# kianoosh-j/CL_MultiView_Stereo

Hardware: AMD Instinct MI355X
Metric: Mpix/s depth (1080p, 128 depth hyp, 5 views) + depth L1 vs ref (higher is better)
Workload: dtype i8 (NCC: 8-bit intensities as int8 v_dot4 operands, i32 window sums, f32 costs; SLIC / superpixel SAD / refinement in f32 with the reference's f64 promotions)

## Files before the change

cl_multiview_stereo_amd/csrc/ncc_mfma.hip:

```cpp
#include <type_traits>

#include "ncc_common.h"

#ifndef MVS_MFMA_SPLIT
#define MVS_MFMA_SPLIT 1
#endif

namespace mvs {
namespace ncc {
namespace {

struct alignas(128) NccMRec {
  int txmax, tymax;
  int bhp, shp;
  int colo[16];
  int pad0[2];
  unsigned off_lo, off_hi;
  int pad[8];
};
static_assert(sizeof(NccMRec) == 4 * kRecWords, "one 128-B record per (chunk, neighbour)");

template <int K, int BW, bool TAIL, bool VERT, int NDB, int NB, int DBG = 0>
__global__ __launch_bounds__(512) __attribute__((amdgpu_waves_per_eu(4))) void k_ncc_mfma(
    const uint2* __restrict__ stats, const uint2* __restrict__ pk, const NccMRec* __restrict__ plan, NccArgs a,
    WtaOut wo) {
  static_assert(NDB == 1 || NDB == 2, "one or two 16-level blocks per chunk");
  static_assert(K == 5 || K == 7, "5 x 5 or 7 x 7 windows");
  static_assert(K == 5 || !VERT, "K = 7: horizontal lists only");
  static_assert(VERT || NB == 2 || NB == 3, "the horizontal form is double- or triple-buffered");
  static_assert(VERT || NDB == (K == 5 ? 2 : 1), "horizontal chunks: 32 levels (K = 5), 16 (K = 7: A takes 32 VGPRs)");
  constexpr int R = K / 2, NW = 8, TH = 8, DC = 16 * NDB, NK = K * K;
  constexpr int XB = K == 5 ? 2 : 4, NYB = K == 5 ? TH / 4 : 1, NBL = XB * NYB, MF = K == 5 ? 1 : 2;
  constexpr int BXW = 8 / XB;
  constexpr int BWP = BW + 1;
  constexpr bool SPLIT = MVS_MFMA_SPLIT;
  extern __shared__ __align__(16) uint8_t smem[];
  const int nbuf = (a.pk_pairs + a.st_pairs) * BWP;
  u32x4* nbase = (u32x4*)smem;
  const int band_bytes = max(NB * nbuf * 16, 3 * 16 * kMfMergeStride * 4);
  float* rsn_l = (float*)(smem + band_bytes);
  float* srl = rsn_l + 64 * TH;
  short* colo_l = (short*)(srl + 64 * TH);

  const int tid = threadIdx.x, lane = tid & 63, wave = __builtin_amdgcn_readfirstlane(tid >> 6);
  const int W = a.W, H = a.H;
  const int Hp2 = (H + 1) >> 1;
  const long Pv = (long)W * Hp2 * 2;
  const long P = (long)W * H;
  const int bid = blockIdx.x, grp = bid & 7;
  const int tg = grp * a.tiles_per_xcd + (bid >> 3);
  if (tg >= a.ntiles * a.nref) return;
  const int ref = tg / a.ntiles, tile = tg - ref * a.ntiles;
  const int x0 = (tile % a.tiles_x) * 64;
  const int y0 = (tile / a.tiles_x) * TH;
  const int nn = a.nn[ref], T = a.nch * nn;
  const NccMRec* rec = plan + a.plan[ref];

  const int bhp = K == 5 ? (TH + 4) / 2 : (TH + 8) / 2, shp = TH / 2;
  const long pk_row = 2L * W * min(max((y0 >> 1) - (K == 5 ? 1 : 2) + wave, 0), Hp2 - 1);
  const long st_row = 2L * W * min(max(y0 / 2 + wave, 0), Hp2 - 1);
  struct StepInfo {
    int tx, shp;
    unsigned lo, hi;
  };
  auto load_info = [&](int t, int n) -> StepInfo {
    const NccMRec& e = rec[t];
    return StepInfo{e.txmax, e.shp, e.off_lo, e.off_hi};
  };
  const int lane_x = x0 + lane;
  auto stage_h = [&](const StepInfo& e, int b) {
    if (DBG == 2) return;
    const int span = (e.shp >> 16) & 0xff, nblk = (span + 127) >> 6;
    const unsigned long long vo = (unsigned long long)e.hi << 32 | e.lo;
    u32x4* npk = nbase + b * nbuf + ((wave & 1) ? (e.shp >> 24) : 0);
    u32x4* nst = nbase + b * nbuf + a.pk_pairs * BWP + ((K == 7 && wave >= 2) ? ((e.shp << 16) >> 24) : 0);
    if (wave < shp) {
      const __amdgpu_buffer_rsrc_t rp = buf_rsrc((const char*)pk + vo + 8 * pk_row, 16 * W);
      const __amdgpu_buffer_rsrc_t rs = buf_rsrc((const char*)stats + vo + 8 * st_row, 16 * W);
      for (int cb = 0; cb < nblk; cb++) {
        const int c0 = min(cb * 64, span);
        const int voff = 16 * min(max(lane_x - e.tx + c0, 0), W - 1);
        __builtin_amdgcn_raw_ptr_buffer_load_lds(rp, (lds_ptr_t)(npk + wave * BWP + c0), 16, voff, 0, 0, 0);
        __builtin_amdgcn_raw_ptr_buffer_load_lds(rs, (lds_ptr_t)(nst + wave * BWP + c0), 16, voff, 0, 0, 0);
      }
    } else if (wave < bhp) {
      const __amdgpu_buffer_rsrc_t rp = buf_rsrc((const char*)pk + vo + 8 * pk_row, 16 * W);
      for (int cb = 0; cb < nblk; cb++) {
        const int c0 = min(cb * 64, span);
        const int voff = 16 * min(max(lane_x - e.tx + c0, 0), W - 1);
        __builtin_amdgcn_raw_ptr_buffer_load_lds(rp, (lds_ptr_t)(npk + wave * BWP + c0), 16, voff, 0, 0, 0);
      }
    }
  };
  auto stage = [&](int t, int n, int b) {
    if (DBG == 2) return;
    const NccMRec& e = rec[t];
    const int span = (e.shp >> 16) & 0xff, nblk = (span + 127) >> 6;
    const long vo = (long)a.view[ref][n] * Pv;
    u32x4* npk = nbase + b * nbuf;
    u32x4* nst = npk + a.pk_pairs * BWP;
    const int xb0 = x0 - e.txmax + lane;
    if constexpr (!VERT) {
      for (int cb = 0; cb < nblk; cb++) {
        const int c0 = min(cb * 64, span);
        const int xx = min(max(xb0 + c0, 0), W - 1);
        if (wave < bhp) glds_b128(pk + vo + pk_row + 2 * xx, npk + wave * BWP + c0);
        if (wave < shp) glds_b128(stats + vo + st_row + 2 * xx, nst + wave * BWP + c0);
      }
    } else {
      const int ebh = e.bhp, esh = e.shp & 0xff;
      const int pm0 = (y0 - R - e.tymax) >> 1, sm0 = (y0 - e.tymax) >> 1;
      for (int cb = 0; cb < nblk; cb++) {
        const int c0 = min(cb * 64, span);
        const int xx = min(max(xb0 + c0, 0), W - 1);
        const uint2* gpk = pk + vo + 2 * xx;
        const uint2* gst = stats + vo + 2 * xx;
        for (int i = wave; i < ebh; i += NW) glds_b128(gpk + 2L * W * min(max(pm0 + i, 0), Hp2 - 1), npk + i * BWP + c0);
        for (int i = wave; i < esh; i += NW) glds_b128(gst + 2L * W * min(max(sm0 + i, 0), Hp2 - 1), nst + i * BWP + c0);
      }
    }
  };

  for (int i = tid; i < T * DC / 2; i += NW * 64) ((int*)colo_l)[i] = rec[i / (DC / 2)].colo[i % (DC / 2)];
  auto nmod = [&](int v) { return v >= nn ? v - nn : v; };
  StepInfo cur{}, nxt{}, nx2{};
  if constexpr (!VERT) {
    cur = load_info(0, 0);
    if (T > 1) nxt = load_info(1, nmod(1 % nn));
    if (NB == 3 && T > 2) nx2 = load_info(2, nmod(2 % nn));
    stage_h(cur, 0);
    if (NB == 3 && T > 1) stage_h(nxt, 1);
  } else {
    stage(0, 0, 0);
  }
  const long zo = (long)a.z[ref] * Pv;
  const int zp0 = min(max((y0 >> 1) - (K == 5 ? 1 : 2), 0), Hp2 - 1);
  const __amdgpu_buffer_rsrc_t rz = buf_rsrc((const char*)pk + 8 * (zo + 2L * W * zp0), 16 * W * min(Hp2 - zp0, 8));
  for (int o = wave; o < TH; o += NW) {
    const int x = x0 + lane, y = y0 + o;
    const int xoff = 16 * min(x, W - 1);
    int s1 = 0, s2 = 0;
#pragma unroll
    for (int k = 0; k < 2 * R + 1; k++) {
      const int yc = min(max(y - R + k, 0), H - 1);
      const u32x2 v = __builtin_amdgcn_raw_buffer_load_b64(rz, xoff, 16 * W * ((yc >> 1) - zp0) + 8 * (yc & 1), 0);
      const unsigned lo = v.x, hi = v.y & (K == 5 ? 0xffu : 0xffffffu);
      s1 = dot4(lo, 0x01010101u, dot4(hi, 0x01010101u, s1));
      s2 = dot4(lo, lo, dot4(hi, hi, s2));
    }
    const bool valid = x - R >= 0 && x + R < W && y - R >= 0 && y + R < H;
    const int var = NK * s2 - s1 * s1;
    srl[lane * TH + o] = !valid ? __int_as_float(0x7fc00000) : (var != 0 ? 1.0f / sqrtf((float)var) : 0.0f);
    rsn_l[lane * TH + o] = -(float)s1;
  }
  i32x4 A[NBL][MF];
  {
    const int mA = lane & 15, g = lane >> 4;
    const int xxA = K == 5 ? mA >> 2 : mA >> 3, yyA = K == 5 ? mA & 3 : mA & 7;
    const unsigned long long cm = (K == 5 ? 0xFFFFFFFFFFull : 0xFFFFFFFFFFFFFFull) << (8 * xxA);
    const unsigned cm_lo = (unsigned)cm, cm_hi = (unsigned)(cm >> 32);
    unsigned msk[MF][4];
#pragma unroll
    for (int mf = 0; mf < MF; mf++)
#pragma unroll
      for (int h = 0; h < 2; h++) {
        const int rr = 2 * (g + 4 * mf) + h;
        const bool in = (unsigned)(rr - yyA - (K == 5 ? 0 : 1)) <= (unsigned)(K - 1);
        msk[mf][2 * h] = in ? cm_lo : 0u;
        msk[mf][2 * h + 1] = in ? cm_hi : 0u;
      }
    constexpr int NPR = K == 5 ? NYB : MF;
    int roff[NPR];
#pragma unroll
    for (int i = 0; i < NPR; i++) {
      const int pr = min(max((K == 5 ? (y0 >> 1) - 1 + 2 * i : (y0 >> 1) - 2 + 4 * i) + g, 0), Hp2 - 1);
      roff[i] = 16 * W * (pr - zp0);
    }
#pragma unroll
    for (int xb = 0; xb < XB; xb++) {
      const int xcol = min(x0 + 8 * wave + BXW * xb, W - 1);
#pragma unroll
      for (int yb = 0; yb < NYB; yb++)
#pragma unroll
        for (int mf = 0; mf < MF; mf++) {
          const u32x4 v = __builtin_amdgcn_raw_buffer_load_b128(rz, roff[K == 5 ? yb : mf], 16 * xcol, 0);
          A[xb * NYB + yb][mf] = i32x4{(int)(v.x & msk[mf][0]), (int)(v.y & msk[mf][1]), (int)(v.z & msk[mf][2]),
                                       (int)(v.w & msk[mf][3])};
        }
    }
  }
  auto pcol = [&](int xb, int g) { return BXW * xb + (K == 5 ? g : g >> 1); };
  auto prow = [&](int yb, int g) { return K == 5 ? 4 * yb : 4 * (g & 1); };
  __syncthreads();

  float E[NBL][NDB][4];
  float wv0[NBL][4], wv1[NBL][4];
  unsigned wi0p[NBL][2];
#pragma unroll
  for (int k = 0; k < NBL; k++) {
#pragma unroll
    for (int r = 0; r < 4; r++) {
      wv0[k][r] = kWtaInit;
      wv1[k][r] = kWtaInit;
    }
    wi0p[k][0] = wi0p[k][1] = 0xffffffffu;
  }
  const i32x4 bias = i32x4{kMagicI, kMagicI, kMagicI, kMagicI};

  auto fold = [&](int c) {
    const int ln = lane_now();
    float kill[NDB];
#pragma unroll
    for (int db = 0; db < NDB; db++) kill[db] = 0.0f;
    if (TAIL && c == a.nch - 1)
#pragma unroll
      for (int db = 0; db < NDB; db++) kill[db] = c * DC + 16 * db + (ln & 15) >= a.D ? INFINITY : 0.0f;
#pragma unroll
    for (int xb = 0; xb < XB; xb++)
#pragma unroll
      for (int yb = 0; yb < NYB; yb++) {
        const int kb = xb * NYB + yb;
        const f32x4 sq = *(const f32x4*)(srl + (8 * wave + pcol(xb, ln >> 4)) * TH + prow(yb, ln >> 4));
        const int dl0 = c * DC + (ln & 15);
        const unsigned d0 = (unsigned)dl0 * 0x10001u, d1 = (unsigned)(dl0 + 16) * 0x10001u;
#pragma unroll
        for (int r = 0; r < 4; r += 2) {
          f32x2 cst[NDB];
#pragma unroll
          for (int db = 0; db < NDB; db++) {
            f32x2 e;
            e.x = __fmul_rn(E[kb][db][r], sq[r]);
            e.y = __fmul_rn(E[kb][db][r + 1], sq[r + 1]);
            if constexpr (NDB == 2) {
              cst[db].x = __fsub_rn(1.0f, e.x);
              cst[db].y = __fsub_rn(1.0f, e.y);
            } else {
              cst[db].x = __fsub_rn(1.0f, vmax_m1(e.x));
              cst[db].y = __fsub_rn(1.0f, vmax_m1(e.y));
            }
            if (TAIL) {
              cst[db].x = __fadd_rn(cst[db].x, kill[db]);
              cst[db].y = __fadd_rn(cst[db].y, kill[db]);
            }
          }
#pragma unroll
          for (int h = 0; h < 2; h++) {
            const unsigned hm = h ? 0xffff0000u : 0x0000ffffu;
            unsigned& wp = wi0p[kb][r >> 1];
            float& v0 = wv0[kb][r + h];
            float& v1 = wv1[kb][r + h];
            if constexpr (NDB == 2) {
              const float c0 = cst[0][h], c1 = cst[NDB - 1][h];
              const float lo = vmin3(c0, c1, INFINITY);
              const float hi = vmaximum3(c0, c1, c1);
              const unsigned idx = lo == c0 ? d0 : d1;
              v1 = vmin3(vmax(v0, lo), v1, hi);
              wp = lo < v0 ? (wp & ~hm) | (idx & hm) : wp;
              v0 = vmin(v0, lo);
            } else {
              const float cc = cst[0][h];
              v1 = vmed3(v0, v1, cc);
              wp = cc < v0 ? (wp & ~hm) | (d0 & hm) : wp;
              v0 = vmin(v0, cc);
            }
          }
        }
      }
  };

  int bt = 0;
  auto step = [&](int t, int n, int cprev, auto first) {
    constexpr bool FIRST = decltype(first)::value;
    const int n1 = n + 1 == nn ? 0 : n + 1;
    StepInfo pf{};
    if constexpr (!VERT) {
      const int n2 = n1 + 1 == nn ? 0 : n1 + 1;
      if (t + NB < T) pf = load_info(t + NB, NB == 2 ? n2 : nmod(n2 + 1));
    }
    if (NB == 1 && t > 0) {
      stage(t, n, 0);
      __syncthreads();
    }
    u32x4* const nbuf_t = nbase + (NB == 2 ? (t & 1) : NB == 3 ? bt : 0) * nbuf;
    if (K == 5 && (VERT || x0 < a.txmax_all)) {
      const int jf = (VERT ? rec[t].txmax : cur.tx) - x0 - 1;
      const int esh = VERT ? rec[t].shp : cur.shp;
      if (jf >= 0 && jf + 1 < 64 + ((esh >> 16) & 0xff)) {
        if (tid < a.pk_pairs) {
          u32x4* e = nbuf_t + tid * BWP + jf + ((tid & 1) ? (esh >> 24) : 0);
          const u32x4 v = e[1];
          *e = u32x4{v.x << 8, (v.y << 8) | (v.x >> 24), v.z << 8, (v.w << 8) | (v.z >> 24)};
        }
        __syncthreads();
      }
    }
    int pieces = 0;
    if constexpr (!VERT && NB == 2) {
      if (t + 1 < T) stage_h(nxt, (t + 1) & 1);
    } else if constexpr (!VERT) {
      if (t + 2 < T) {
        stage_h(nx2, bt == 0 ? 2 : bt - 1);
        const int nb2 = (((nx2.shp >> 16) & 0xff) + 127) >> 6;
        pieces = (wave < bhp ? nb2 : 0) + (wave < shp ? nb2 : 0);
      }
    } else {
      if (NB == 2 && t + 1 < T) stage(t + 1, n1, (t + 1) & 1);
    }
    if (FIRST && cprev >= 0) fold(cprev);
    const u32x4* npk = nbuf_t;
    const u32x4* nst = npk + a.pk_pairs * BWP;
    const int ln = lane_now();
    const int g = ln >> 4;
    int cl[NDB], iB0[NDB], iB1[NDB], iS0[NDB], iS1[NDB];
#pragma unroll
    for (int db = 0; db < NDB; db++) {
      const int v = colo_l[t * DC + 16 * db + (ln & 15)];
      if constexpr (!VERT) {
        cl[db] = v;
      } else {
        const int col = 8 * wave + (v & 0xff), o = v >> 8;
        const int r0 = o + 2 * g, r1 = r0 + 1, s1 = o + 1;
        iB0[db] = 2 * ((r0 >> 1) * BWP + col) + (r0 & 1);
        iB1[db] = 2 * ((r1 >> 1) * BWP + col) + (r1 & 1);
        iS0[db] = 4 * ((o >> 1) * BWP + col + g) + (o & 1);
        iS1[db] = 4 * ((s1 >> 1) * BWP + col + g) + (s1 & 1);
      }
    }
    const int sg = (!VERT && (g & 1)) ? (cur.shp >> 24) : 0;
    const int tg = (K == 7 && (g & 1)) ? ((cur.shp << 16) >> 24) : 0;
    auto bread = [&](int xb, int yb, int db, int mf) -> i32x4 {
      if constexpr (!VERT) {
        const int pr = K == 5 ? 2 * yb + g : g + 4 * mf;
        return __builtin_bit_cast(i32x4, npk[pr * BWP + 8 * wave + BXW * xb + cl[db] + sg]);
      } else {
        const uint2* b2 = (const uint2*)npk;
        const int off = 2 * (2 * yb * BWP + 4 * xb);
        const uint2 lo = b2[iB0[db] + off], hi = b2[iB1[db] + off];
        return i32x4{(int)lo.x, (int)lo.y, (int)hi.x, (int)hi.y};
      }
    };
    auto sread = [&](int xb, int yb, int db, f32x4& s0, f32x4& s1) {
      if constexpr (!VERT) {
        const int colS = 8 * wave + pcol(xb, g) + cl[db] + tg;
        const int sp = prow(yb, g) >> 1;
        s0 = __builtin_bit_cast(f32x4, nst[sp * BWP + colS]);
        s1 = __builtin_bit_cast(f32x4, nst[(sp + 1) * BWP + colS]);
      } else {
        const float* f = (const float*)nst;
        const int off = 4 * (2 * yb * BWP + 4 * xb);
        const int q0 = iS0[db] + off, q1 = iS1[db] + off, q2 = q0 + 4 * BWP, q3 = q1 + 4 * BWP;
        s0 = f32x4{f[q0], f[q1], f[q0 + 2], f[q1 + 2]};
        s1 = f32x4{f[q2], f[q3], f[q2 + 2], f[q3 + 2]};
      }
    };
    auto finish = [&](int xb, int yb, int db, const i32x4& acc, const f32x4& nsr, const f32x4& s0,
                      const f32x4& s1) {
#pragma unroll
      for (int p = 0; p < 2; p++) {
        const f32x4 sv = p ? s1 : s0;
        f32x2 xv;
        xv.x = __fmaf_rn(nsr[2 * p], sv.z, __fmul_rn(__fsub_rn(__int_as_float(acc[2 * p]), kMagicF), sv.x));
        xv.y = __fmaf_rn(nsr[2 * p + 1], sv.w, __fmul_rn(__fsub_rn(__int_as_float(acc[2 * p + 1]), kMagicF), sv.y));
        const int kb = xb * NYB + yb;
        if (FIRST) {
          E[kb][db][2 * p] = xv.x;
          E[kb][db][2 * p + 1] = xv.y;
        } else {
          E[kb][db][2 * p] = vmax(E[kb][db][2 * p], xv.x);
          E[kb][db][2 * p + 1] = vmax(E[kb][db][2 * p + 1], xv.y);
        }
      }
    };
#pragma unroll
    for (int k = 0; k < (DBG == 1 ? 0 : NBL); k++) {
      const int xb = k / NYB, yb = k % NYB;
      const f32x4 nsr = *(const f32x4*)(rsn_l + (8 * wave + pcol(xb, g)) * TH + prow(yb, g));
#pragma unroll
      for (int db = 0; db < NDB; db++) {
        i32x4 bv[MF];
#pragma unroll
        for (int mf = 0; mf < MF; mf++) bv[mf] = bread(xb, yb, db, mf);
        f32x4 s0, s1;
        sread(xb, yb, db, s0, s1);
        if (SPLIT) __builtin_amdgcn_sched_barrier(0);
        i32x4 acc = __builtin_amdgcn_mfma_i32_16x16x64_i8(A[k][0], bv[0], bias, 0, 0, 0);
        if constexpr (MF == 2) acc = __builtin_amdgcn_mfma_i32_16x16x64_i8(A[k][1], bv[1], acc, 0, 0, 0);
        finish(xb, yb, db, acc, nsr, s0, s1);
      }
    }
    if constexpr (!VERT && NB == 3) {
      wait_vm_barrier(pieces);
    } else {
      __syncthreads();
    }
    if constexpr (!VERT) {
      cur = nxt;
      if constexpr (NB == 3) {
        nxt = nx2;
        nx2 = pf;
        bt = bt == 2 ? 0 : bt + 1;
      } else {
        nxt = pf;
      }
    }
  };
  {
    int t = 0;
    for (int c = 0; c < a.nch; c++) {
      step(t++, 0, c - 1, std::true_type{});
      for (int n = 1; n < nn; n++) step(t++, n, -1, std::false_type{});
    }
  }
  fold(a.nch - 1);

  float* m0 = (float*)smem;
  float* m1 = m0 + 16 * kMfMergeStride;
  int* mi = (int*)(m1 + 16 * kMfMergeStride);
#pragma unroll
  for (int yb = 0; yb < TH / 4; yb++) {
    {
      const int ln = lane_now(), cls = ln & 15, g = ln >> 4;
      const int kyb = K == 5 ? yb : 0;
      if (K == 5 || (g & 1) == yb) {
#pragma unroll
        for (int xb = 0; xb < XB; xb++)
#pragma unroll
          for (int r = 0; r < 4; r++) {
            const int kb = xb * NYB + kyb;
            const int q = cls * kMfMergeStride + r * 64 + 8 * wave + pcol(xb, g);
            const unsigned v = (r & 1) ? wi0p[kb][r >> 1] >> 16 : wi0p[kb][r >> 1] & 0xffffu;
            m0[q] = wv0[kb][r];
            m1[q] = wv1[kb][r];
            mi[q] = (int)v;
          }
      }
    }
    __syncthreads();
    if (tid < 256) {
      const int q = tid, xx = x0 + (q & 63), yy = y0 + 4 * yb + (q >> 6);
      float v0s[16], v1s[16];
      unsigned is[16];
#pragma unroll
      for (int w = 0; w < 16; w++) {
        v0s[w] = m0[w * kMfMergeStride + q];
        is[w] = (unsigned)mi[w * kMfMergeStride + q];
        v1s[w] = m1[w * kMfMergeStride + q];
      }
      const float bv = vmin16(v0s);
      unsigned ti[16];
#pragma unroll
      for (int w = 0; w < 16; w++) ti[w] = v0s[w] == bv ? is[w] : 0xffffffffu;
      const unsigned bi = vmin16u(ti);
      const unsigned bl = bi - 1u;
      float sv[16];
#pragma unroll
      for (int w = 0; w < 16; w++) sv[w] = is[w] - bl <= 2u ? v1s[w] : v0s[w];
      float c2 = vmin16(sv);
      const bool all2 = !(bv < 2.0f);
      const int b = (int)bi;
      if (!all2 && a.D > min(b + 1, a.D - 1) - max(b - 1, 0) + 1) c2 = vmin(c2, 2.0f);
      if (xx < W && yy < H) {
        const long p = P * ref + (long)yy * W + xx;
        wo.disp[p] = a.D <= 0 ? 0.0f : wo.levels[all2 ? 0 : b];
        if (wo.conf) wo.conf[p] = (all2 || c2 == kWtaInit) ? 0.0f : c2 - bv;
      }
    }
    __syncthreads();
  }
}


template <int K, int BW, bool TAIL, bool VERT, int NDB, int NB, int DBG = 0>
int launch_mfma_bw(const NccCall& c) {
  auto kern = k_ncc_mfma<K, BW, TAIL, VERT, NDB, NB, DBG>;
  MVS_HIP(raise_lds(c.ctx, (const void*)kern, c.L.lds), "hipFuncSetAttribute(ncc mfma lds)");
  const auto ev = kernel_events(c.ctx);
  hipExtLaunchKernelGGL(kern, dim3(8 * c.L.args.tiles_per_xcd), dim3(512), c.L.lds, c.ctx->stream, ev.first, ev.second,
                        0, c.stats, c.pk, (const NccMRec*)c.plan, c.L.args, c.wo);
  MVS_LAUNCH_CHECK("k_ncc_mfma (fused WTA)");
  return 0;
}

template <bool TAIL, int NDB, int NB>
int launch_vert(const NccCall& c) {
  switch (c.L.BW) {
    case 80: return launch_mfma_bw<5, 80, TAIL, true, NDB, NB>(c);
    case 96: return launch_mfma_bw<5, 96, TAIL, true, NDB, NB>(c);
    case 128: return launch_mfma_bw<5, 128, TAIL, true, NDB, NB>(c);
  }
  return no_kernel();
}

template <int DBG>
int launch_probe(const NccCall& c) {
  const NccLaunch& L = c.L;
  if (L.TAIL || L.NB != 2) return no_kernel();
  if (L.K == 7 && !L.VERT && L.BW == 128 && L.NDB == 1) return launch_mfma_bw<7, 128, false, false, 1, 2, DBG>(c);
  if (L.K == 5 && !L.VERT && L.BW == 192 && L.NDB == 2) return launch_mfma_bw<5, 192, false, false, 2, 2, DBG>(c);
  if (L.K == 5 && L.VERT && L.BW == 80 && L.NDB == 1) return launch_mfma_bw<5, 80, false, true, 1, 2, DBG>(c);
  return no_kernel();
}

}

int launch_ncc_mfma(const NccCall& c) {
  const NccLaunch& L = c.L;
  if (L.DBG) return L.DBG == 1 ? launch_probe<1>(c) : launch_probe<2>(c);
  if (L.VERT) {
    if (L.K != 5) return no_kernel();
    const int form = 10 * L.NDB + L.NB;
    if (form == 22) return L.TAIL ? launch_vert<true, 2, 2>(c) : launch_vert<false, 2, 2>(c);
    if (form == 21) return L.TAIL ? launch_vert<true, 2, 1>(c) : launch_vert<false, 2, 1>(c);
    if (form == 12) return L.TAIL ? launch_vert<true, 1, 2>(c) : launch_vert<false, 1, 2>(c);
    if (form == 11) return L.TAIL ? launch_vert<true, 1, 1>(c) : launch_vert<false, 1, 1>(c);
    return no_kernel();
  }
  if (L.K == 7 && L.NDB == 1) {
    if (L.TAIL) return L.BW == 192 && L.NB == 2 ? launch_mfma_bw<7, 192, true, false, 1, 2>(c) : no_kernel();
    if (L.BW == 128 && L.NB == 3) return launch_mfma_bw<7, 128, false, false, 1, 3>(c);
    if (L.BW == 128 && L.NB == 2) return launch_mfma_bw<7, 128, false, false, 1, 2>(c);
    return L.BW == 192 && L.NB == 2 ? launch_mfma_bw<7, 192, false, false, 1, 2>(c) : no_kernel();
  }
  if (L.K != 5 || L.NDB != 2 || L.NB != 2) return no_kernel();
  if (L.TAIL) return L.BW == 192 ? launch_mfma_bw<5, 192, true, false, 2, 2>(c) : no_kernel();
  if (L.BW == 128) return launch_mfma_bw<5, 128, false, false, 2, 2>(c);
  return L.BW == 192 ? launch_mfma_bw<5, 192, false, false, 2, 2>(c) : no_kernel();
}

}
}
```

Baseline: 6141.

## Interleave WTA fold into first MFMA step and software-pipeline LDS reads

Moves the per-chunk winner-take-all fold from a separate pass into the first step of the next chunk, where it is interleaved block by block with the MFMA loads and compute. It also rotates the non-first steps into a software pipeline: the LDS reads for the next block are issued right after the current MFMA, and the per-element finishes are split, so LDS latency overlaps with matrix work. Scheduling barriers and empty asm register pins enforce this order. The costs are higher register pressure at waves_per_eu(4) and a rigid schedule the compiler can no longer rearrange.

After: 6197, median of 6. No clear change (+0.9%).

```diff
diff --git a/cl_multiview_stereo_amd/csrc/ncc_mfma.hip b/cl_multiview_stereo_amd/csrc/ncc_mfma.hip
--- a/cl_multiview_stereo_amd/csrc/ncc_mfma.hip
+++ b/cl_multiview_stereo_amd/csrc/ncc_mfma.hip
@@ -1,14 +1,20 @@
 #include <type_traits>
 
 #include "ncc_common.h"
-
-#ifndef MVS_MFMA_SPLIT
-#define MVS_MFMA_SPLIT 1
-#endif
 
 namespace mvs {
 namespace ncc {
 namespace {
+
+__device__ __forceinline__ void pin_order() {
+  asm volatile("" ::: "memory");
+  __builtin_amdgcn_sched_barrier(0);
+}
+__device__ __forceinline__ void keep(float& a, float& b) { asm volatile("" : "+v"(a), "+v"(b)); }
+__device__ __forceinline__ void keep(unsigned& a) { asm volatile("" : "+v"(a)); }
+enum { kStepMax, kStepFirst, kStepFold };
+constexpr bool kFoldUnder = true;
+constexpr bool kRotate = true;
 
 struct alignas(128) NccMRec {
   int txmax, tymax;
@@ -33,7 +39,6 @@
   constexpr int XB = K == 5 ? 2 : 4, NYB = K == 5 ? TH / 4 : 1, NBL = XB * NYB, MF = K == 5 ? 1 : 2;
   constexpr int BXW = 8 / XB;
   constexpr int BWP = BW + 1;
-  constexpr bool SPLIT = MVS_MFMA_SPLIT;
   extern __shared__ __align__(16) uint8_t smem[];
   const int nbuf = (a.pk_pairs + a.st_pairs) * BWP;
   u32x4* nbase = (u32x4*)smem;
@@ -207,70 +212,76 @@
   }
   const i32x4 bias = i32x4{kMagicI, kMagicI, kMagicI, kMagicI};
 
+  auto fold_sq = [&](int kb, int g) -> f32x4 {
+    return *(const f32x4*)(srl + (8 * wave + pcol(kb / NYB, g)) * TH + prow(kb % NYB, g));
+  };
+  auto fold_block = [&](int c, int kb, const f32x4& sq, auto last, const float (&kill)[NDB]) {
+    constexpr bool KILL = TAIL && decltype(last)::value;
+    const int dl0 = c * DC + (lane_now() & 15);
+    const unsigned d0 = (unsigned)dl0 * 0x10001u, d1 = (unsigned)(dl0 + 16) * 0x10001u;
+#pragma unroll
+    for (int r = 0; r < 4; r += 2) {
+      f32x2 cst[NDB];
+#pragma unroll
+      for (int db = 0; db < NDB; db++) {
+        f32x2 e;
+        e.x = __fmul_rn(E[kb][db][r], sq[r]);
+        e.y = __fmul_rn(E[kb][db][r + 1], sq[r + 1]);
+        if constexpr (NDB == 2) {
+          cst[db].x = __fsub_rn(1.0f, e.x);
+          cst[db].y = __fsub_rn(1.0f, e.y);
+        } else {
+          cst[db].x = __fsub_rn(1.0f, vmax_m1(e.x));
+          cst[db].y = __fsub_rn(1.0f, vmax_m1(e.y));
+        }
+        if (KILL) {
+          cst[db].x = __fadd_rn(cst[db].x, kill[db]);
+          cst[db].y = __fadd_rn(cst[db].y, kill[db]);
+        }
+      }
+#pragma unroll
+      for (int h = 0; h < 2; h++) {
+        const unsigned hm = h ? 0xffff0000u : 0x0000ffffu;
+        unsigned& wp = wi0p[kb][r >> 1];
+        float& v0 = wv0[kb][r + h];
+        float& v1 = wv1[kb][r + h];
+        if constexpr (NDB == 2) {
+          const float c0 = cst[0][h], c1 = cst[NDB - 1][h];
+          const float lo = vmin3(c0, c1, INFINITY);
+          const float hi = vmaximum3(c0, c1, c1);
+          const unsigned idx = lo == c0 ? d0 : d1;
+          v1 = vmin3(vmax(v0, lo), v1, hi);
+          wp = lo < v0 ? (wp & ~hm) | (idx & hm) : wp;
+          v0 = vmin(v0, lo);
+        } else {
+          const float cc = cst[0][h];
+          v1 = vmed3(v0, v1, cc);
+          wp = cc < v0 ? (wp & ~hm) | (d0 & hm) : wp;
+          v0 = vmin(v0, cc);
+        }
+      }
+      keep(wv0[kb][r], wv0[kb][r + 1]);
+      keep(wv1[kb][r], wv1[kb][r + 1]);
+      keep(wi0p[kb][r >> 1]);
+    }
+  };
+  const float kill0[NDB] = {};
   auto fold = [&](int c) {
-    const int ln = lane_now();
     float kill[NDB];
 #pragma unroll
     for (int db = 0; db < NDB; db++) kill[db] = 0.0f;
     if (TAIL && c == a.nch - 1)
 #pragma unroll
-      for (int db = 0; db < NDB; db++) kill[db] = c * DC + 16 * db + (ln & 15) >= a.D ? INFINITY : 0.0f;
-#pragma unroll
-    for (int xb = 0; xb < XB; xb++)
-#pragma unroll
-      for (int yb = 0; yb < NYB; yb++) {
-        const int kb = xb * NYB + yb;
-        const f32x4 sq = *(const f32x4*)(srl + (8 * wave + pcol(xb, ln >> 4)) * TH + prow(yb, ln >> 4));
-        const int dl0 = c * DC + (ln & 15);
-        const unsigned d0 = (unsigned)dl0 * 0x10001u, d1 = (unsigned)(dl0 + 16) * 0x10001u;
-#pragma unroll
-        for (int r = 0; r < 4; r += 2) {
-          f32x2 cst[NDB];
-#pragma unroll
-          for (int db = 0; db < NDB; db++) {
-            f32x2 e;
-            e.x = __fmul_rn(E[kb][db][r], sq[r]);
-            e.y = __fmul_rn(E[kb][db][r + 1], sq[r + 1]);
-            if constexpr (NDB == 2) {
-              cst[db].x = __fsub_rn(1.0f, e.x);
-              cst[db].y = __fsub_rn(1.0f, e.y);
-            } else {
-              cst[db].x = __fsub_rn(1.0f, vmax_m1(e.x));
-              cst[db].y = __fsub_rn(1.0f, vmax_m1(e.y));
-            }
-            if (TAIL) {
-              cst[db].x = __fadd_rn(cst[db].x, kill[db]);
-              cst[db].y = __fadd_rn(cst[db].y, kill[db]);
-            }
-          }
-#pragma unroll
-          for (int h = 0; h < 2; h++) {
-            const unsigned hm = h ? 0xffff0000u : 0x0000ffffu;
-            unsigned& wp = wi0p[kb][r >> 1];
-            float& v0 = wv0[kb][r + h];
-            float& v1 = wv1[kb][r + h];
-            if constexpr (NDB == 2) {
-              const float c0 = cst[0][h], c1 = cst[NDB - 1][h];
-              const float lo = vmin3(c0, c1, INFINITY);
-              const float hi = vmaximum3(c0, c1, c1);
-              const unsigned idx = lo == c0 ? d0 : d1;
-              v1 = vmin3(vmax(v0, lo), v1, hi);
-              wp = lo < v0 ? (wp & ~hm) | (idx & hm) : wp;
-              v0 = vmin(v0, lo);
-            } else {
-              const float cc = cst[0][h];
-              v1 = vmed3(v0, v1, cc);
-              wp = cc < v0 ? (wp & ~hm) | (d0 & hm) : wp;
-              v0 = vmin(v0, cc);
-            }
-          }
-        }
-      }
+      for (int db = 0; db < NDB; db++) kill[db] = c * DC + 16 * db + (lane_now() & 15) >= a.D ? INFINITY : 0.0f;
+    const int g = lane_now() >> 4;
+#pragma unroll
+    for (int kb = 0; kb < NBL; kb++) fold_block(c, kb, fold_sq(kb, g), std::true_type{}, kill);
   };
 
   int bt = 0;
-  auto step = [&](int t, int n, int cprev, auto first) {
-    constexpr bool FIRST = decltype(first)::value;
+  auto step = [&](int t, int n, int cprev, auto mode) {
+    constexpr bool FIRST = decltype(mode)::value != kStepMax;
+    constexpr bool FOLD = decltype(mode)::value == kStepFold && DBG != 1 && kFoldUnder;
     const int n1 = n + 1 == nn ? 0 : n + 1;
     StepInfo pf{};
     if constexpr (!VERT) {
@@ -306,7 +317,7 @@
     } else {
       if (NB == 2 && t + 1 < T) stage(t + 1, n1, (t + 1) & 1);
     }
-    if (FIRST && cprev >= 0) fold(cprev);
+    if (decltype(mode)::value == kStepFold && !FOLD) fold(cprev);
     const u32x4* npk = nbuf_t;
     const u32x4* nst = npk + a.pk_pairs * BWP;
     const int ln = lane_now();
@@ -339,53 +350,96 @@
         return i32x4{(int)lo.x, (int)lo.y, (int)hi.x, (int)hi.y};
       }
     };
-    auto sread = [&](int xb, int yb, int db, f32x4& s0, f32x4& s1) {
+    auto sread = [&](int xb, int yb, int db, int p) -> f32x4 {
       if constexpr (!VERT) {
         const int colS = 8 * wave + pcol(xb, g) + cl[db] + tg;
         const int sp = prow(yb, g) >> 1;
-        s0 = __builtin_bit_cast(f32x4, nst[sp * BWP + colS]);
-        s1 = __builtin_bit_cast(f32x4, nst[(sp + 1) * BWP + colS]);
+        return __builtin_bit_cast(f32x4, nst[(sp + p) * BWP + colS]);
       } else {
         const float* f = (const float*)nst;
-        const int off = 4 * (2 * yb * BWP + 4 * xb);
-        const int q0 = iS0[db] + off, q1 = iS1[db] + off, q2 = q0 + 4 * BWP, q3 = q1 + 4 * BWP;
-        s0 = f32x4{f[q0], f[q1], f[q0 + 2], f[q1 + 2]};
-        s1 = f32x4{f[q2], f[q3], f[q2 + 2], f[q3 + 2]};
+        const int off = 4 * ((2 * yb + p) * BWP + 4 * xb);
+        const int q0 = iS0[db] + off, q1 = iS1[db] + off;
+        return f32x4{f[q0], f[q1], f[q0 + 2], f[q1 + 2]};
       }
     };
-    auto finish = [&](int xb, int yb, int db, const i32x4& acc, const f32x4& nsr, const f32x4& s0,
-                      const f32x4& s1) {
-#pragma unroll
-      for (int p = 0; p < 2; p++) {
-        const f32x4 sv = p ? s1 : s0;
-        f32x2 xv;
-        xv.x = __fmaf_rn(nsr[2 * p], sv.z, __fmul_rn(__fsub_rn(__int_as_float(acc[2 * p]), kMagicF), sv.x));
-        xv.y = __fmaf_rn(nsr[2 * p + 1], sv.w, __fmul_rn(__fsub_rn(__int_as_float(acc[2 * p + 1]), kMagicF), sv.y));
-        const int kb = xb * NYB + yb;
-        if (FIRST) {
-          E[kb][db][2 * p] = xv.x;
-          E[kb][db][2 * p + 1] = xv.y;
+    auto nread = [&](int k) -> f32x4 {
+      return *(const f32x4*)(rsn_l + (8 * wave + pcol(k / NYB, g)) * TH + prow(k % NYB, g));
+    };
+    auto mfma = [&](int k, const i32x4 (&bv)[MF]) -> i32x4 {
+      i32x4 acc = __builtin_amdgcn_mfma_i32_16x16x64_i8(A[k][0], bv[0], bias, 0, 0, 0);
+      if constexpr (MF == 2) acc = __builtin_amdgcn_mfma_i32_16x16x64_i8(A[k][1], bv[1], acc, 0, 0, 0);
+      return acc;
+    };
+    auto finish = [&](int kb, int db, int p, const i32x4& acc, const f32x4& nsr, const f32x4& sv) {
+      f32x2 xv;
+      xv.x = __fmaf_rn(nsr[2 * p], sv.z, __fmul_rn(__fsub_rn(__int_as_float(acc[2 * p]), kMagicF), sv.x));
+      xv.y = __fmaf_rn(nsr[2 * p + 1], sv.w, __fmul_rn(__fsub_rn(__int_as_float(acc[2 * p + 1]), kMagicF), sv.y));
+      if (FIRST) {
+        E[kb][db][2 * p] = xv.x;
+        E[kb][db][2 * p + 1] = xv.y;
+        keep(E[kb][db][2 * p], E[kb][db][2 * p + 1]);
+      } else {
+        E[kb][db][2 * p] = vmax(E[kb][db][2 * p], xv.x);
+        E[kb][db][2 * p + 1] = vmax(E[kb][db][2 * p + 1], xv.y);
+      }
+    };
+    constexpr int NI = DBG == 1 ? 0 : NBL * NDB;
+    if constexpr (FIRST || !kRotate || (VERT && NDB == 2)) {
+      f32x4 nsr;
+#pragma unroll
+      for (int i = 0; i < NI; i++) {
+        const int k = i / NDB, db = i % NDB, xb = k / NYB, yb = k % NYB;
+        i32x4 bv[MF];
+        f32x4 s0, s1;
+        auto breads = [&]() {
+#pragma unroll
+          for (int mf = 0; mf < MF; mf++) bv[mf] = bread(xb, yb, db, mf);
+        };
+        auto sreads = [&]() {
+          if (db == 0) nsr = nread(k);
+          s0 = sread(xb, yb, db, 0);
+          s1 = sread(xb, yb, db, 1);
+        };
+        if (db == 0 && FOLD) {
+          const f32x4 sq = fold_sq(k, g);
+          breads();
+          sreads();
+          pin_order();
+          fold_block(cprev, k, sq, std::false_type{}, kill0);
         } else {
-          E[kb][db][2 * p] = vmax(E[kb][db][2 * p], xv.x);
-          E[kb][db][2 * p + 1] = vmax(E[kb][db][2 * p + 1], xv.y);
+          breads();
+          sreads();
         }
-      }
-    };
-#pragma unroll
-    for (int k = 0; k < (DBG == 1 ? 0 : NBL); k++) {
-      const int xb = k / NYB, yb = k % NYB;
-      const f32x4 nsr = *(const f32x4*)(rsn_l + (8 * wave + pcol(xb, g)) * TH + prow(yb, g));
-#pragma unroll
-      for (int db = 0; db < NDB; db++) {
-        i32x4 bv[MF];
-#pragma unroll
-        for (int mf = 0; mf < MF; mf++) bv[mf] = bread(xb, yb, db, mf);
-        f32x4 s0, s1;
-        sread(xb, yb, db, s0, s1);
-        if (SPLIT) __builtin_amdgcn_sched_barrier(0);
-        i32x4 acc = __builtin_amdgcn_mfma_i32_16x16x64_i8(A[k][0], bv[0], bias, 0, 0, 0);
-        if constexpr (MF == 2) acc = __builtin_amdgcn_mfma_i32_16x16x64_i8(A[k][1], bv[1], acc, 0, 0, 0);
-        finish(xb, yb, db, acc, nsr, s0, s1);
+        pin_order();
+        const i32x4 acc = mfma(k, bv);
+        finish(k, db, 0, acc, nsr, s0);
+        finish(k, db, 1, acc, nsr, s1);
+        pin_order();
+      }
+    } else if constexpr (NI > 0) {
+      i32x4 bv[MF];
+      f32x4 nsr = nread(0), s0, s1;
+#pragma unroll
+      for (int mf = 0; mf < MF; mf++) bv[mf] = bread(0, 0, 0, mf);
+      s0 = sread(0, 0, 0, 0);
+      s1 = sread(0, 0, 0, 1);
+#pragma unroll
+      for (int i = 0; i < NI; i++) {
+        const int k = i / NDB, db = i % NDB;
+        const int k1 = (i + 1) / NDB, db1 = (i + 1) % NDB, xb1 = k1 / NYB, yb1 = k1 % NYB;
+        const bool more = i + 1 < NI;
+        pin_order();
+        const i32x4 acc = mfma(k, bv);
+        if (more)
+#pragma unroll
+          for (int mf = 0; mf < MF; mf++) bv[mf] = bread(xb1, yb1, db1, mf);
+        pin_order();
+        finish(k, db, 0, acc, nsr, s0);
+        if (more) s0 = sread(xb1, yb1, db1, 0);
+        pin_order();
+        finish(k, db, 1, acc, nsr, s1);
+        if (more) s1 = sread(xb1, yb1, db1, 1);
+        if (more && k1 != k) nsr = nread(k1);
       }
     }
     if constexpr (!VERT && NB == 3) {
@@ -406,9 +460,11 @@
   };
   {
     int t = 0;
-    for (int c = 0; c < a.nch; c++) {
-      step(t++, 0, c - 1, std::true_type{});
-      for (int n = 1; n < nn; n++) step(t++, n, -1, std::false_type{});
+    step(t++, 0, -1, std::integral_constant<int, kStepFirst>{});
+    for (int n = 1; n < nn; n++) step(t++, n, -1, std::integral_constant<int, kStepMax>{});
+    for (int c = 1; c < a.nch; c++) {
+      step(t++, 0, c - 1, std::integral_constant<int, kStepFold>{});
+      for (int n = 1; n < nn; n++) step(t++, n, -1, std::integral_constant<int, kStepMax>{});
     }
   }
   fold(a.nch - 1);
```
